# url-kaist/Quatro

Hardware: NVIDIA H100
Metric: registrations/sec (64-ring pair) (higher is better)
Workload: dtype f32 (front end, match, graph filter) / f64 (graph boundary, GNC, COTE)

## Files before the change

quatro_b200/capi.py:

```python
from __future__ import annotations

import ctypes as C
from typing import Optional, Sequence

import numpy as np

from . import _build

PMC_EXACT, PMC_HEU, KCORE_HEU, INLIER_NONE = 0, 1, 2, 3
FLAG_CLIQUE_TRUNCATED = 1
FLAG_LISTS_TRUNCATED = 2
COTE_MEDIAN, COTE_WEIGHTED_MEAN = 0, 1
MEM_HOST, MEM_DEVICE = 0, 1

STATUS_NAMES = {0: "OK", 1: "DEGENERATE_CLIQUE", 2: "DEGENERATE_INPUT", 3: "CAPACITY_EXCEEDED", -1: "ERR_BAD_ARG",
                -2: "ERR_NO_DEVICE", -3: "ERR_CUDA", -4: "ERR_UNSUPPORTED", -5: "ERR_VOXEL_OVERFLOW"}


class Params(C.Structure):
    _fields_ = [
        ("voxel_size", C.c_float), ("normal_radius", C.c_float), ("fpfh_radius", C.c_float), ("grid_cell", C.c_float),
        ("tuple_scale", C.c_float), ("use_crosscheck", C.c_int32), ("use_tuple_test", C.c_int32),
        ("tuple_trials_per_corr", C.c_int32), ("skip_flagged", C.c_int32), ("reserved0", C.c_int32),
        ("seed", C.c_uint64),
# ... 946 lines not shown
    def register_batch_raw(self, pair_array, n: int, params: Params, kind: int, out: np.ndarray):
        return self._check(self.lib.qb200_register_batch(self.h, pair_array, n, C.byref(params), kind, _ptr(out)), "qb200_register_batch")

    def register_batch_enqueue_raw(self, pair_array, n: int, params: Params, kind: int, out: np.ndarray):
        return self._check(self.lib.qb200_register_batch_enqueue(self.h, pair_array, n, C.byref(params), kind, _ptr(out)), "qb200_register_batch_enqueue")

    def register_batch_flush(self):
        return self._check(self.lib.qb200_register_batch_flush(self.h), "qb200_register_batch_flush")

    def last_clique(self, cap: int = 1 << 16):
        idx = np.zeros(cap, np.int32)
        n = C.c_int32(0)
        self._check(self.lib.qb200_get_last_clique(self.h, _ptr(idx), cap, C.byref(n)), "qb200_get_last_clique")
        return idx[: n.value].copy()

    def last_final_inliers(self, cap: int = 1 << 16):
        idx = np.zeros(cap, np.int32)
        n = C.c_int32(0)
        self._check(self.lib.qb200_get_last_final_inliers(self.h, _ptr(idx), cap, C.byref(n)), "qb200_get_last_final_inliers")
        return idx[: n.value].copy()

    def last_correspondences(self, cap: int = 1 << 16):
        corr = np.zeros((cap, 2), np.int32)
        sm = np.zeros((cap, 4), np.float32)
        tm = np.zeros((cap, 4), np.float32)
        n = C.c_int32(0)
        self._check(self.lib.qb200_get_last_correspondences(self.h, _ptr(corr), _ptr(sm), _ptr(tm), cap, C.byref(n)),
                    "qb200_get_last_correspondences")
        return corr[: n.value].copy(), sm[: n.value].copy(), tm[: n.value].copy()

    def debug_match_stats(self, reset: bool = True) -> dict:
        out = np.zeros(4, np.uint64)
        self._check(self.lib.qb200_debug_match_stats(self.h, _ptr(out), int(reset)), "qb200_debug_match_stats")
        return {"exact_evals": int(out[0]), "tiles": int(out[1]), "warmups": int(out[2]), "aborted_stripes": int(out[3])}

    def debug_nn_tables(self, n_src: int, n_tgt: int):
        rb, cb = np.full(n_src, ~np.uint64(0)), np.full(n_tgt, ~np.uint64(0))
        self._check(self.lib.qb200_debug_nn_tables(self.h, _ptr(rb), n_src, _ptr(cb), n_tgt), "qb200_debug_nn_tables")
        return rb, cb

    def debug_tc_profile(self, reset: bool = True) -> np.ndarray:
        out = np.zeros(24, np.uint64)
        self._check(self.lib.qb200_debug_tc_profile(self.h, _ptr(out), int(reset)), "qb200_debug_tc_profile")
        return out

    def debug_tc_footprint(self) -> dict:
        out = np.zeros(5, np.int32)
        self._check(self.lib.qb200_debug_tc_footprint(self.h, _ptr(out)), "qb200_debug_tc_footprint")
        return {"threads": int(out[0]), "dyn_smem": int(out[1]), "static_smem": int(out[2]), "regs": int(out[3]),
                "ctas_per_sm": int(out[4])}

    def debug_match_verify(self, reset: bool = True) -> dict:
        out = np.zeros(2, np.uint64)
        self._check(self.lib.qb200_debug_match_verify(self.h, _ptr(out), int(reset)), "qb200_debug_match_verify")
        return {"compared": int(out[0]), "mismatches": int(out[1])}

    def debug_tc_distances(self, a33, b33) -> np.ndarray:
        a33, b33 = _f32(a33, 33), _f32(b33, 33)
        out = np.zeros((128, 128), np.float32)
        self._check(self.lib.qb200_debug_tc_distances(self.h, _ptr(a33), len(a33), _ptr(b33), len(b33), _ptr(out)), "qb200_debug_tc_distances")
        return out[: len(a33), : len(b33)].copy()

    def kernel_ms(self):
        ms = np.zeros(2, np.float32)
        calls = np.zeros(2, np.int32)
        self.lib.qb200_get_kernel_ms(self.h, _ptr(ms), _ptr(calls), 2)
        return ms, calls
# ... 6 lines not shown
```

quatro_b200/csrc/common.cuh:

```cuda
#pragma once
#include <cuda_runtime.h>
#include <stdint.h>
#include <stdio.h>

#include "quatro_b200.h"

namespace qb {

constexpr int kOffIJ = 1 << 17;
constexpr int kOffK = 1 << 15;
constexpr uint64_t kCellMask = (1ull << 52) - 1;
constexpr uint64_t kCellInvalid = kCellMask;
constexpr int kCloudShift = 52;

__host__ __device__ __forceinline__ bool cell_ok(int i, int j, int k) {
  return i >= -kOffIJ && i < kOffIJ - 1 && j >= -kOffIJ && j < kOffIJ - 1 && k >= -kOffK && k < kOffK - 1;
}
__host__ __device__ __forceinline__ uint64_t cell_key(int i, int j, int k) {
  return ((uint64_t)(k + kOffK) << 36) | ((uint64_t)(j + kOffIJ) << 18) | (uint64_t)(i + kOffIJ);
}

constexpr int kVoxShift = 31;
constexpr uint64_t kVoxMask = (1ull << kVoxShift) - 1;
constexpr uint64_t kVoxInvalid = kVoxMask;
constexpr int kVsChunks = 64;
constexpr int kVsTile = 2048;

__device__ __forceinline__ bool raw_point_kept(const float4 p, int skip_flagged) {
  return isfinite(p.x) && isfinite(p.y) && isfinite(p.z) && !(skip_flagged && p.w < 0.0f);
}
__host__ __device__ __forceinline__ int vox_chunk_size(int n) { return n > 0 ? (n + kVsChunks - 1) / kVsChunks : 1; }

constexpr int kDescDim = 33;
constexpr int kDescPad = 36;
constexpr int kDescK = 40;
constexpr int kMatchTile = 128;
constexpr int kNbrGlobalCap = 80;

struct WaveCounters {
  int* n_valid;
  int* n_vox;
  int* n_lat;
  int* n_cells;
  int* cloud_status;
  int* bbox;
  int* vox_digits;
  int* n_mutual;
  int* n_corr;
  int* swapped;
  int* n_clique;
  int* max_core;
  int* n_final;
  int* flags;
  long long* n_edges;
};

#define QB_CUDA_TRY(h, expr)                                                                    \
  do {                                                                                          \
    cudaError_t _e = (expr);                                                                    \
    if (_e != cudaSuccess) {                                                                    \
      (h)->fail(__FILE__, __LINE__, cudaGetErrorString(_e));                                    \
      return QB200_ERR_CUDA;                                                                    \
    }                                                                                           \
  } while (0)

__device__ __forceinline__ int float_ordered(float f) {
  const int i = __float_as_int(f);
  return i >= 0 ? i : i ^ 0x7FFFFFFF;
// ... 81 lines not shown
```

quatro_b200/csrc/match.cu:

```cuda
#include <stdlib.h>

#include "handle.cuh"
#include "qb_math.cuh"

namespace qb {

constexpr int kMT = kMatchTile;
constexpr int kMatchThreads = 256;

__device__ __forceinline__ unsigned long long pack_dist(float d, int idx) {
  return ((unsigned long long)__float_as_uint(d) << 32) | (unsigned)idx;
}
__device__ __forceinline__ unsigned long long umin64(unsigned long long a, unsigned long long b) { return a < b ? a : b; }
__device__ __forceinline__ unsigned long long shfl_xor_u64(unsigned long long v, int m) {
  const unsigned lo = __shfl_xor_sync(0xffffffffu, (unsigned)v, m), hi = __shfl_xor_sync(0xffffffffu, (unsigned)(v >> 32), m);
  return ((unsigned long long)hi << 32) | lo;
}

__device__ __forceinline__ void cp_async16(void* smem, const void* gmem) {
  const unsigned s = (unsigned)__cvta_generic_to_shared(smem);
  asm volatile("cp.async.cg.shared.global [%0], [%1], 16;\n" ::"r"(s), "l"(gmem));
}
__device__ __forceinline__ void cp_async_commit() { asm volatile("cp.async.commit_group;\n" ::); }
template <int N>
// ... 29 lines not shown
  load_tile_async(Bs0, B, V, 0);
  cp_async_commit();

  unsigned long long rbest[8];
#pragma unroll
  for (int r = 0; r < 8; ++r) rbest[r] = ~0ull;

  const int n_tiles = (nB + kMT - 1) / kMT;
  for (int jt = 0; jt < n_tiles; ++jt) {
    float(*Bs)[kMT] = (jt & 1) ? Bs1 : Bs0;
    if (jt + 1 < n_tiles) {
      load_tile_async((jt & 1) ? Bs0 : Bs1, B, V, (jt + 1) * kMT);
      cp_async_commit();
      cp_async_wait<1>();
    } else {
      cp_async_wait<0>();
    }
    __syncthreads();

    float acc[8][8];
#pragma unroll
    for (int r = 0; r < 8; ++r)
#pragma unroll
      for (int c = 0; c < 8; ++c) acc[r][c] = 0.0f;
#pragma unroll 3
    for (int d = 0; d < kDescDim; ++d) {
      const float4 a0 = *reinterpret_cast<const float4*>(&As[d][ty * 8]), a1 = *reinterpret_cast<const float4*>(&As[d][ty * 8 + 4]);
      const float4 b0 = *reinterpret_cast<const float4*>(&Bs[d][tx * 8]), b1 = *reinterpret_cast<const float4*>(&Bs[d][tx * 8 + 4]);
      const float a[8] = {a0.x, a0.y, a0.z, a0.w, a1.x, a1.y, a1.z, a1.w};
      const float b[8] = {b0.x, b0.y, b0.z, b0.w, b1.x, b1.y, b1.z, b1.w};
#pragma unroll
      for (int r = 0; r < 8; ++r)
#pragma unroll
        for (int c = 0; c < 8; ++c) {
          const float diff = a[r] - b[c];
          acc[r][c] = __fmaf_rn(diff, diff, acc[r][c]);
        }
    }
    const int cbase = jt * kMT + tx * 8, rbase = r0 + ty * 8;
    unsigned long long cbest[8];
#pragma unroll
    for (int c = 0; c < 8; ++c) cbest[c] = ~0ull;
#pragma unroll
    for (int r = 0; r < 8; ++r) {
      const bool rv = rbase + r < nA;
#pragma unroll
      for (int c = 0; c < 8; ++c) {
        const float dd = acc[r][c];
        const bool ok = rv && (cbase + c < nB) && (dd == dd);
        const unsigned long long pr = ok ? pack_dist(dd, cbase + c) : ~0ull;
        const unsigned long long pc = ok ? pack_dist(dd, rbase + r) : ~0ull;
        rbest[r] = umin64(rbest[r], pr);
        cbest[c] = umin64(cbest[c], pc);
      }
    }
#pragma unroll
    for (int c = 0; c < 8; ++c) cbest[c] = umin64(cbest[c], shfl_xor_u64(cbest[c], 16));
    if ((threadIdx.x & 31) < 16) {
#pragma unroll
      for (int c = 0; c < 8; ++c) colred[warp][tx * 8 + c] = cbest[c];
    }
    __syncthreads();
    if (threadIdx.x < kMT) {
      unsigned long long m = colred[0][threadIdx.x];
#pragma unroll
      for (int w = 1; w < 8; ++w) m = umin64(m, colred[w][threadIdx.x]);
      const int col = jt * kMT + threadIdx.x;
      if (col < nB && m != ~0ull) atomicMin(colbest + (size_t)pair * V + col, m);
    }
  }
// ... 368 lines not shown
```

quatro_b200/csrc/tc_match.cu:

```cuda
#include "handle.cuh"
#include <cstdlib>

namespace qb {

constexpr int kTcM = 128, kTcN = 64;
constexpr int kTcBlk = 64;
constexpr int kTcKB = kDescK / 8;
constexpr int kTcTileBytes = kDescK * kTcBlk * 4;
constexpr int kTileFloats = kDescK * kTcBlk;
constexpr int kTcImages = 3;
constexpr int kTcEpiWarps = 8;
constexpr int kTcThreads = (kTcEpiWarps + 2) * 32;
constexpr int kTcDone = 4;
constexpr int kTcStages = 2;
constexpr int kTcSmemTiles = 256;
constexpr float kTcC = 1.2e-4f;
constexpr float kTcNormMax = 0x1p124f;
constexpr float kTcNormRel = 4.0e-6f;
constexpr int kSpinLimit = 400000;

__device__ __forceinline__ uint32_t smem_u32(const void* p) { return (uint32_t)__cvta_generic_to_shared(p); }

__device__ __forceinline__ uint64_t tc_smem_desc(uint32_t addr) {
  return (uint64_t)((addr & 0x3FFFF) >> 4) | ((uint64_t)((kTcBlk * 16) >> 4) << 16) | ((uint64_t)(128 >> 4) << 32);
}

__device__ __forceinline__ void wgmma_tf32_64x64x8(float (&d)[32], uint64_t adesc, uint64_t bdesc, int accumulate) {
  asm volatile(
      "{\n\t"
      ".reg .pred p;\n\t"
      "setp.ne.b32 p, %34, 0;\n\t"
      "wgmma.mma_async.sync.aligned.m64n64k8.f32.tf32.tf32 "
      "{%0, %1, %2, %3, %4, %5, %6, %7, %8, %9, %10, %11, %12, %13, %14, %15, "
      "%16, %17, %18, %19, %20, %21, %22, %23, %24, %25, %26, %27, %28, %29, %30, %31}, %32, %33, p, 1, 1;\n\t"
      "}\n"
      : "+f"(d[0]), "+f"(d[1]), "+f"(d[2]), "+f"(d[3]), "+f"(d[4]), "+f"(d[5]), "+f"(d[6]), "+f"(d[7]), "+f"(d[8]), "+f"(d[9]),
        "+f"(d[10]), "+f"(d[11]), "+f"(d[12]), "+f"(d[13]), "+f"(d[14]), "+f"(d[15]), "+f"(d[16]), "+f"(d[17]), "+f"(d[18]),
        "+f"(d[19]), "+f"(d[20]), "+f"(d[21]), "+f"(d[22]), "+f"(d[23]), "+f"(d[24]), "+f"(d[25]), "+f"(d[26]), "+f"(d[27]),
        "+f"(d[28]), "+f"(d[29]), "+f"(d[30]), "+f"(d[31])
      : "l"(adesc), "l"(bdesc), "r"(accumulate)
      : "memory");
}

__device__ __forceinline__ bool wg_all(bool v, int g) {
  uint32_t r;
  asm volatile(
      "{\n\t.reg .pred p, q;\n\t"
      "setp.ne.u32 p, %1, 0;\n\t"
      "bar.red.and.pred q, %2, 128, p;\n\t"
      "selp.u32 %0, 1, 0, q;\n\t}\n"
      : "=r"(r)
      : "r"((uint32_t)v), "r"(1 + g)
// ... 119 lines not shown
  else rowbest[(size_t)pair * V + q] = rowbest_u[(size_t)pair * V + u];
}

__device__ __forceinline__ void mbar_init(uint32_t bar, int count) {
  asm volatile("mbarrier.init.shared::cta.b64 [%0], %1;\n" ::"r"(bar), "r"(count) : "memory");
}
__device__ __forceinline__ void mbar_expect_tx(uint32_t bar, uint32_t bytes) {
  asm volatile("mbarrier.arrive.expect_tx.shared::cta.b64 _, [%0], %1;\n" ::"r"(bar), "r"(bytes) : "memory");
}
__device__ __forceinline__ void bulk_g2s(uint32_t dst, const void* src, uint32_t bytes, uint32_t bar) {
  asm volatile("cp.async.bulk.shared::cluster.global.mbarrier::complete_tx::bytes [%0], [%1], %2, [%3];\n" ::"r"(dst), "l"(src), "r"(bytes),
               "r"(bar)
               : "memory");
}
__device__ __forceinline__ bool mbar_wait(uint32_t bar, uint32_t parity) {
  for (int spin = 0; spin < kSpinLimit; ++spin) {
    uint32_t ok;
    asm volatile(
        "{\n\t.reg .pred p;\n\t"
        "mbarrier.try_wait.parity.shared::cta.b64 p, [%1], %2;\n\t"
        "selp.u32 %0, 1, 0, p;\n\t}\n"
        : "=r"(ok)
        : "r"(bar), "r"(parity)
        : "memory");
    if (ok) return true;
  }
  return false;
}

__device__ __forceinline__ unsigned long long tc_pack(float d, int idx) {
  return ((unsigned long long)__float_as_uint(d) << 32) | (unsigned)idx;
}

__device__ __forceinline__ void mbar_arrive(uint32_t bar) {
  asm volatile("mbarrier.arrive.shared::cta.b64 _, [%0];\n" ::"r"(bar) : "memory");
}
__device__ __forceinline__ unsigned tc_fkey(float f) {
  unsigned key = __float_as_uint(f);
  key = (key & 0x80000000u) ? ~key : (key | 0x80000000u);
  return f == f ? key : 0xFFFFFFFFu;
}
__device__ __forceinline__ float tc_fkey_inv(unsigned key) { return __uint_as_float((key & 0x80000000u) ? (key & 0x7FFFFFFFu) : ~key); }

template <bool kDbg, bool kProf = false>
__global__ void __launch_bounds__(kTcThreads, 2)
tc_nn_kernel(const float* __restrict__ tiles, const float* __restrict__ norm, const int* __restrict__ n_vox, int V,
             const uint32_t* __restrict__ perm, unsigned long long* __restrict__ rowbest, unsigned long long* __restrict__ colbest_r,
             unsigned* __restrict__ tile_cmax, int* __restrict__ fallback, unsigned long long* __restrict__ stats,
             float* __restrict__ dbg_tile) {
  extern __shared__ __align__(128) unsigned char smem[];
  __shared__ uint64_t s_fullx[kTcStages], s_sfree[kTcStages], s_fullhl, s_mma[kTcDone], s_afull;
  __shared__ unsigned long long s_rbest[kTcM];
  __shared__ __align__(16) float s_wcj[kTcEpiWarps][kTcN];
  __shared__ unsigned short s_queue[kTcEpiWarps][32];
  __shared__ int s_seq[8];
  __shared__ float s_tlb[kTcSmemTiles];
  __shared__ int s_dead, s_abort, s_evals, s_warm, s_npos;
  __shared__ int s_ndec;

  const int pair = blockIdx.y, stripe = blockIdx.x;
  const int cloudA = 2 * pair, cloudB = 2 * pair + 1;
  const int nA = n_vox[cloudA], nB = n_vox[cloudB];
  const int r0 = stripe * kTcM;
  if (r0 >= nA || nB <= 0) return;

  const int warp = threadIdx.x >> 5, lane = threadIdx.x & 31;
  const int NB = V / kTcBlk;
  auto tick = [&]() -> long long { return kProf ? clock64() : 0ll; };
  auto prof = [&](int slot, long long cyc) { if (kProf && lane == 0) atomicAdd(stats + slot, (unsigned long long)cyc); };
  const long long t_begin = tick();
  constexpr uint32_t kABytes = (kTcM / kTcBlk) * kTcImages * kTcTileBytes;
  constexpr uint32_t kHLBytes = 2 * kTcTileBytes;
  constexpr uint32_t kXBytes = kTcTileBytes;
  const uint32_t sA = smem_u32(smem), sHL = sA + kABytes, sX0 = sHL + kHLBytes;
  const float* __restrict__ tA = tiles + (size_t)cloudA * NB * kTcImages * kTileFloats;
  const float* __restrict__ tB = tiles + (size_t)cloudB * NB * kTcImages * kTileFloats;
  const float* __restrict__ nrmA = norm + (size_t)cloudA * V;
  const float* __restrict__ nrmB = norm + (size_t)cloudB * V;
  const uint32_t* __restrict__ permA = perm + (size_t)cloudA * V;
  const uint32_t* __restrict__ permB = perm + (size_t)cloudB * V;
  unsigned long long* __restrict__ cbg = colbest_r + (size_t)pair * V;
  const uint32_t bar_fullx0 = smem_u32(&s_fullx[0]), bar_sfree0 = smem_u32(&s_sfree[0]), bar_fullhl = smem_u32(&s_fullhl),
                 bar_mma0 = smem_u32(&s_mma[0]), bar_a = smem_u32(&s_afull);
  const int n_tiles = (nB + kTcN - 1) / kTcN;

  if (threadIdx.x == 0) {
    for (int i = 0; i < kTcStages; ++i) { mbar_init(bar_fullx0 + 8 * i, 1); mbar_init(bar_sfree0 + 8 * i, kTcEpiWarps); }
    mbar_init(bar_fullhl, 1);
    for (int i = 0; i < kTcDone; ++i) mbar_init(bar_mma0 + 8 * i, kTcEpiWarps);
    mbar_init(bar_a, 1);
    s_dead = 0; s_abort = 0; s_evals = 0; s_warm = 0; s_npos = 0; s_ndec = 0;
    asm volatile("fence.mbarrier_init.release.cluster;\n" ::: "memory");
  }
  if (threadIdx.x < kTcM) s_rbest[threadIdx.x] = ~0ull;
  __syncthreads();
  const long long t_setup = tick();
  if (kProf && threadIdx.x == 0) { atomicAdd(stats + 8, 1ull); atomicAdd(stats + 10, (unsigned long long)(t_setup - t_begin)); }
  volatile int* v_dead = &s_dead;
  volatile int* v_abort = &s_abort;
  volatile int* v_seq = s_seq;
  volatile int* v_ndec = &s_ndec;
  auto wait_decided = [&](int n) -> bool {
    for (int spin = 0; spin < kSpinLimit; ++spin) {
      if (*v_ndec > n) { __threadfence_block(); return true; }
      __nanosleep(32);
    }
    return false;
  };
  volatile unsigned long long* v_rbest = s_rbest;

  if (warp == kTcEpiWarps) {
    auto issue_hl = [&](int n) {
      const int t = v_seq[n & 7];
      if (lane != 0) return;
      if (t < 0) { mbar_arrive(bar_fullhl); return; }
      mbar_expect_tx(bar_fullhl, kHLBytes);
      bulk_g2s(sHL, tB + (size_t)t * kTcImages * kTileFloats, kHLBytes, bar_fullhl);
    };
    if (lane == 0) {
      mbar_expect_tx(bar_a, kABytes);
      bulk_g2s(sA, tA + (size_t)stripe * (kTcM / kTcBlk) * kTcImages * kTileFloats, kABytes, bar_a);
    }
    bool ok = wait_decided(0);
    if (ok) issue_hl(0);
    long long p_wm = 0, p_wd = 0;
    bool ended = !ok || v_seq[0] < 0;
    for (int k = 0; ok && !ended; ++k) {
// ... 9 lines not shown
    }
    prof(12, p_wm); prof(28, p_wd);
    if (!ok) *v_dead = 1;
  } else if (warp == kTcEpiWarps + 1) {
    const float amin = sqrtf(nrmA[r0]), amax = sqrtf(nrmA[(r0 + kTcM < nA ? r0 + kTcM : nA) - 1]);
    auto tile_lb = [&](int t) -> float {
      const float bmin = sqrtf(nrmB[t * kTcN]), bmax = sqrtf(nrmB[(t * kTcN + kTcN < nB ? t * kTcN + kTcN : nB) - 1]);
      const float gap = fmaxf(amin - bmax, bmin - amax) - (2.0e-3f + kTcNormRel * (amax + bmax));
      if (!(amin <= amax && bmin <= bmax)) return 0.0f;
      return gap > 0.0f ? gap * gap * 0.9999f : 0.0f;
    };
    constexpr int kPq = kTcSmemTiles / 32;
    const uint2* __restrict__ tcm2 = reinterpret_cast<const uint2*>(tile_cmax) + (size_t)pair * (V / kTcN);
    uint2 pq[kPq];
    auto fetch_tcm = [&]() {
#pragma unroll
      for (int i = 0; i < kPq; ++i) pq[i] = lane + 32 * i < n_tiles ? __ldcg(tcm2 + lane + 32 * i) : make_uint2(0xFFFFFFFFu, 0xFFFFFFFFu);
    };
    fetch_tcm();
    int t0 = 0;
    {
      float best = INFINITY;
      for (int t = lane; t < n_tiles; t += 32) {
        const float g = tile_lb(t);
        if (t < kTcSmemTiles) s_tlb[t] = g;
        if (g < best) { best = g; t0 = t; }
      }
      const unsigned key = __reduce_min_sync(0xffffffffu, tc_fkey(best));
      const unsigned who = __ballot_sync(0xffffffffu, tc_fkey(best) == key);
      t0 = __shfl_sync(0xffffffffu, t0, __ffs(who) - 1);
      __syncwarp();
    }
    auto tlb = [&](int t) -> float { return t < kTcSmemTiles ? s_tlb[t] : tile_lb(t); };
    int lo = t0 - 1, hi = t0 + 1;
    bool first = true, done = false;
    auto next_tile = [&]() -> int {
      if (first) { first = false; return t0; }
      unsigned rmax = 0;
#pragma unroll
      for (int i = 0; i < kTcM / 32; ++i) {
        const int row = lane + 32 * i;
        if (r0 + row < nA) {
          const unsigned long long rb = v_rbest[row];
          rmax = max(rmax, rb == ~0ull ? 0x7F800000u : (unsigned)(rb >> 32));
        }
      }
      const float rmaxf = __uint_as_float(__reduce_max_sync(0xffffffffu, rmax));
      unsigned tcm[kPq];
#pragma unroll
      for (int i = 0; i < kPq; ++i) tcm[i] = max(pq[i].x, pq[i].y);
      if (*v_abort || *v_dead) return -1;
      const bool is_left = lane < 16;
      while (true) {
        if (lo < 0 && hi >= n_tiles) return -1;
        const int t = is_left ? lo - lane : hi + (lane - 16);
        const bool valid = is_left ? t >= 0 : t < n_tiles;
        const float lb = valid ? tlb(t) : INFINITY;
        unsigned cm = 0xFFFFFFFFu;
        {
          const int src = t & 31, sl = (t >> 5) & (kPq - 1);
#pragma unroll
          for (int i = 0; i < kPq; ++i) {
            const unsigned a = __shfl_sync(0xffffffffu, tcm[i], src);
            if (sl == i) cm = a;
          }
          if (!valid) cm = 0xFFFFFFFFu;
          else if (t >= kTcSmemTiles) { const uint2 q = __ldcg(tcm2 + t); cm = max(q.x, q.y); }
        }
        const bool visit = valid && (lb <= 0.0f || !(lb > rmaxf) || !(lb > __uint_as_float(cm)));
        const unsigned vb = __ballot_sync(0xffffffffu, visit);
// ... 2 lines not shown
        if (fl == 16 && fr == 16) { lo -= 16; hi += 16; continue; }
        const float gl = __shfl_sync(0xffffffffu, lb, fl & 15), gh = __shfl_sync(0xffffffffu, lb, 16 + (fr & 15));
        const bool left = fr == 16 || (fl < 16 && gl <= gh);
        const int tv = left ? lo - fl : hi + fr;
        lo -= left ? fl + 1 : fl;
        hi += left ? fr : fr + 1;
        return tv;
      }
    };
    int n_issued = 0;
    auto decide = [&](int n) {
      int t = -1;
      if (!done) {
        t = next_tile();
        if (t < 0) done = true; else ++n_issued;
      }
      if (lane == 0) {
        v_seq[n & 7] = t;
        __threadfence_block();
        *v_ndec = n + 1;
      }
      __syncwarp();
      if (!done) fetch_tcm();
      return t;
    };
    auto issue_x = [&](int n) {
      const int t = v_seq[n & 7];
      if (lane != 0) return;
      const uint32_t bar = bar_fullx0 + 8 * (n % kTcStages);
      if (t < 0) { mbar_arrive(bar); return; }
      mbar_expect_tx(bar, kXBytes);
      bulk_g2s(sX0 + (n % kTcStages) * kXBytes, tB + ((size_t)t * kTcImages + 2) * kTileFloats, kXBytes, bar);
    };
    for (int n = 0; n < 3; ++n) {
      decide(n);
      if (n < kTcStages) issue_x(n);
    }
    prof(11, tick() - t_setup);
    long long p_wm = 0, p_dec = 0, p_sf = 0;
    auto mbar_test = [&](uint32_t bar, uint32_t parity) -> bool {
      uint32_t ready;
      asm volatile(
          "{\n\t.reg .pred p;\n\t"
          "mbarrier.test_wait.parity.shared::cta.b64 p, [%1], %2;\n\t"
          "selp.u32 %0, 1, 0, p;\n\t}\n"
          : "=r"(ready)
          : "r"(bar), "r"(parity)
          : "memory");
      return __all_sync(0xffffffffu, ready != 0);
    };
    int nd = 3, nx = kTcStages;
    bool ok = true, end_decided = v_seq[0] < 0 || v_seq[1] < 0 || v_seq[2] < 0;
    int idle = 0;
    long long t_idle = 0;
    while (ok && !(end_decided && nx == nd)) {
      const uint32_t bar_s = bar_sfree0 + 8 * (nx % kTcStages), par_s = (uint32_t)((nx / kTcStages - 1) & 1);
      const uint32_t bar_m = bar_mma0 + 8 * ((nd - 3) & (kTcDone - 1)), par_m = (uint32_t)(((nd - 3) >> 2) & 1);
      const bool can_x = nx < nd, can_d = !end_decided && nd < nx + 4;
      if (can_x && mbar_test(bar_s, par_s)) {
        if (kProf && idle) { (can_d ? p_wm : p_sf) += tick() - t_idle; }
        idle = 0;
        issue_x(nx);
        ++nx;
        continue;
      }
      if (can_d && mbar_test(bar_m, par_m)) {
        const long long t1 = tick();
        if (kProf && idle) { (can_x ? p_wm : p_sf) += t1 - t_idle; }
        idle = 0;
        if (decide(nd) < 0) end_decided = true;
        ++nd;
        p_dec += tick() - t1;
        continue;
      }
      if (idle == 0) t_idle = tick();
      if (++idle > kSpinLimit) { ok = false; break; }
      __nanosleep(32);
    }
    prof(29, p_wm); prof(13, p_dec); prof(14, p_sf);
    if (!ok) *v_dead = 1;
    if (lane == 0) s_npos = n_issued;
  } else {
    const int wg = warp >> 2;
    const int rbase = wg * 64 + 16 * (warp & 3);
    const int cl = 2 * (lane & 3);
    const float kLow = 1.0f - 0.5f * kTcC;
    const float kW = kTcC / kLow;
    bool row_ok[2];
    float nam[2], Ri_ub[2];
    unsigned oa[2];
#pragma unroll
    for (int h = 0; h < 2; ++h) {
      const int gi = r0 + rbase + (lane >> 2) + 8 * h;
      row_ok[h] = gi < nA;
      nam[h] = row_ok[h] ? kLow * nrmA[gi] : INFINITY;
      oa[h] = row_ok[h] ? permA[gi] : 0u;
      Ri_ub[h] = row_ok[h] ? INFINITY : -INFINITY;
    }
    const uint32_t row_bits = (row_ok[0] ? 0x33333333u : 0u) | (row_ok[1] ? 0xCCCCCCCCu : 0u);
    const float4* __restrict__ aex = reinterpret_cast<const float4*>(smem + (wg * kTcImages + 2) * kTcTileBytes);
    const uint32_t aH = sA + (uint32_t)(wg * kTcImages * kTcTileBytes), aL = aH + kTcTileBytes;
    float* wcj = s_wcj[warp];
    unsigned short* wq = s_queue[warp];
    int evals_w = 0;
    bool alive = mbar_wait(bar_a, 0);
    const long long t_loop = tick();
    prof(19, t_loop - t_setup);
    long long p_wx = 0, p_wmm = 0, p_ld = 0, p_prep = 0, p_fil = 0, p_ev = 0;
    int p_tiles = 0;
    int pf_tile = -1;
    unsigned long long pf_cb[2] = {~0ull, ~0ull};
    unsigned pf_ob[2] = {0u, 0u};
    unsigned* __restrict__ tcmw = tile_cmax + ((size_t)pair * (V / kTcN)) * 2;
    int rr_tile = -1;
    unsigned rr_val[2] = {0u, 0u};
    auto rr_flush = [&]() {
      if (rr_tile < 0) return;
#pragma unroll
      for (int s = 0; s < 2; ++s) {
        const unsigned m = __reduce_max_sync(0xffffffffu, rr_val[s]);
        if (lane == 0) atomicMin(tcmw + (size_t)rr_tile * 2 + s, m);
      }
      rr_tile = -1;
    };
    for (int k = 0;; ++k) {
      const int ts = k & (kTcDone - 1), st = k % kTcStages;
      const long long q0 = tick();
      if (alive) alive = mbar_wait(bar_fullx0 + 8 * st, (uint32_t)((k / kTcStages) & 1));
      const long long q1 = tick();
      p_wx += q1 - q0;
// ... 38 lines not shown
        break;
      }
      float d[32];
#pragma unroll
      for (int i = 0; i < 32; ++i) d[i] = 0.0f;
      {
        constexpr uint32_t kKB = 2 * kTcBlk * 16;
        const uint32_t bH = sHL, bL = bH + kTcTileBytes;
        asm volatile("wgmma.fence.sync.aligned;\n" ::: "memory");
#pragma unroll
        for (int kb = 0; kb < kTcKB; ++kb) {
          wgmma_tf32_64x64x8(d, tc_smem_desc(aH + kb * kKB), tc_smem_desc(bL + kb * kKB), kb > 0);
          wgmma_tf32_64x64x8(d, tc_smem_desc(aL + kb * kKB), tc_smem_desc(bH + kb * kKB), 1);
        }
#pragma unroll
        for (int kb = 0; kb < kTcKB; ++kb) wgmma_tf32_64x64x8(d, tc_smem_desc(aH + kb * kKB), tc_smem_desc(bH + kb * kKB), 1);
        asm volatile("wgmma.commit_group.sync.aligned;\n" ::: "memory");
        asm volatile("wgmma.wait_group.sync.aligned 0;\n" ::: "memory");
#pragma unroll
        for (int i = 0; i < 32; ++i) asm volatile("" : "+f"(d[i])::"memory");
      }
      __syncwarp();
      if (lane == 0) mbar_arrive(bar_mma0 + 8 * ts);
      const long long q3 = tick();
      p_wmm += q3 - q2;
      p_prep += q2 - q1;
      ++p_tiles;
      const bool skip = __any_sync(0xffffffffu, (*v_abort | *v_dead) != 0);
      const long long q4 = tick();
      p_ld += q4 - q3;
      if (!skip) {
        const float4* __restrict__ bex = reinterpret_cast<const float4*>(smem + kABytes + kHLBytes + st * kXBytes);
        float dbest[2];
        bool col_warm = false;
#pragma unroll
        for (int s = 0; s < 2; ++s) {
          const float nbm = bex[9 * kTcBlk + 32 * s + lane].x;
          dbest[s] = cb_cur[s] == ~0ull ? INFINITY : __uint_as_float((unsigned)(cb_cur[s] >> 32));
          wcj[32 * s + lane] = nbm == INFINITY ? -INFINITY : dbest[s];
          col_warm |= cb_cur[s] == ~0ull && nbm != INFINITY;
        }
        float Ri[2];
        bool row_warm = false;
#pragma unroll
        for (int h = 0; h < 2; ++h) {
          const unsigned long long rb = v_rbest[rbase + (lane >> 2) + 8 * h];
          Ri[h] = fminf(Ri_ub[h], rb == ~0ull ? INFINITY : __uint_as_float((unsigned)(rb >> 32)));
          row_warm |= row_ok[h] && Ri[h] == INFINITY;
        }
        __syncwarp();
        if (__any_sync(0xffffffffu, row_warm || col_warm)) {
          if (lane == 0) atomicAdd(&s_warm, 1);
          float rowub[2] = {INFINITY, INFINITY};
#pragma unroll
          for (int i = 0; i < 32; i += 4) {
#pragma unroll
            for (int e = 0; e < 2; ++e) {
              const int c = 2 * i + cl + e;
              const float nbc = bex[9 * kTcBlk + c].x;
              const float ub0 = fmaf(kW, nam[0] + nbc, d[i + e]), ub1 = fmaf(kW, nam[1] + nbc, d[i + 2 + e]);
              rowub[0] = fminf(rowub[0], ub0);
              rowub[1] = fminf(rowub[1], ub1);
              unsigned mn = min(ub0 >= 0.0f ? __float_as_uint(ub0) : 0xFFFFFFFFu, ub1 >= 0.0f ? __float_as_uint(ub1) : 0xFFFFFFFFu);
              mn = min(mn, __shfl_xor_sync(0xffffffffu, mn, 4));
              mn = min(mn, __shfl_xor_sync(0xffffffffu, mn, 8));
              mn = min(mn, __shfl_xor_sync(0xffffffffu, mn, 16));
              if (lane < 4 && mn != 0xFFFFFFFFu && nbc != INFINITY) wcj[c] = fminf(wcj[c], __uint_as_float(mn));
            }
          }
#pragma unroll
          for (int h = 0; h < 2; ++h) {
            rowub[h] = fminf(rowub[h], __shfl_xor_sync(0xffffffffu, rowub[h], 1));
            rowub[h] = fminf(rowub[h], __shfl_xor_sync(0xffffffffu, rowub[h], 2));
            if (row_ok[h]) { Ri_ub[h] = fminf(Ri_ub[h], rowub[h]); Ri[h] = fminf(Ri[h], Ri_ub[h]); }
          }
        }
        __syncwarp();
        const long long q5 = tick();
        p_prep += q5 - q4;
        const int ncol = nB - c0;
        uint32_t mask = 0, col_bits = 0;
#pragma unroll
        for (int i = 0; i < 32; i += 4) {
          const float2 x = *reinterpret_cast<const float2*>(wcj + 2 * i + cl);
#pragma unroll
          for (int e = 0; e < 4; ++e) {
            const float lbv = d[i + e];
            const float xc = (e & 1) ? x.y : x.x;
            asm("{\n\t.reg .pred p, q;\n\t"
                "setp.le.f32 p, %1, %2;\n\t"
                "setp.le.or.f32 q, %1, %3, p;\n\t"
                "@q or.b32 %0, %0, %4;\n\t}\n"
                : "+r"(mask)
                : "f"(lbv), "f"(xc), "f"(Ri[e >> 1]), "r"(1u << (i + e)));
            if (2 * i + cl + (e & 1) < ncol) col_bits |= 1u << (i + e);
            if (kDbg) {
              const int h = e >> 1, c = 2 * i + cl + (e & 1);
              if (stripe == 0 && row_ok[h] && c < ncol)
                dbg_tile[(size_t)oa[h] * 128 + permB[c0 + c]] = fmaf(0.5f * kW, nam[h] + bex[9 * kTcBlk + c].x, lbv);
            }
          }
        }
        mask &= col_bits & row_bits;
        int remaining = __reduce_add_sync(0xffffffffu, __popc(mask));
        const long long q6 = tick();
        p_fil += q6 - q5;
        evals_w += remaining;
        while (remaining > 0) {
          int tot;
          int p = warp_excl_scan(__popc(mask), &tot);
          while (mask && p < 32) {
            const int i = __ffs(mask) - 1;
            mask &= mask - 1;
            wq[p++] = (unsigned short)((lane << 5) | i);
          }
          __syncwarp();
          const int nb = tot < 32 ? tot : 32;
          const int q = lane < nb ? wq[lane] : 0;
          const int sl = q >> 5, i = q & 31, h = (i >> 1) & 1;
          const int rr = rbase + (sl >> 2) + 8 * h;
          const int c = 8 * (i >> 2) + 2 * (sl & 3) + (i & 1);
          float acc = 0.0f;
#pragma unroll
          for (int kc = 0; kc < (kDescDim + 3) / 4; ++kc) {
            const float4 a = aex[kc * kTcBlk + (rr & (kTcBlk - 1))], b = bex[kc * kTcBlk + c];
            float diff = a.x - b.x;
            acc = __fmaf_rn(diff, diff, acc);
            if (4 * kc + 1 < kDescDim) { diff = a.y - b.y; acc = __fmaf_rn(diff, diff, acc); }
            if (4 * kc + 2 < kDescDim) { diff = a.z - b.z; acc = __fmaf_rn(diff, diff, acc); }
            if (4 * kc + 3 < kDescDim) { diff = a.w - b.w; acc = __fmaf_rn(diff, diff, acc); }
          }
          const float db0 = __shfl_sync(0xffffffffu, dbest[0], c & 31), db1 = __shfl_sync(0xffffffffu, dbest[1], c & 31);
          const unsigned ob0 = __shfl_sync(0xffffffffu, ob[0], c & 31), ob1 = __shfl_sync(0xffffffffu, ob[1], c & 31);
          const unsigned oa0 = __shfl_sync(0xffffffffu, oa[0], sl & ~3), oa1 = __shfl_sync(0xffffffffu, oa[1], sl & ~3);
          const float dbc = c < 32 ? db0 : db1;
          const unsigned oc = c < 32 ? ob0 : ob1;
          const unsigned orow = h ? oa1 : oa0;
          if (lane < nb && acc == acc) {
            const unsigned long long pr = tc_pack(acc, (int)oc);
            if (pr < v_rbest[rr]) atomicMin(&s_rbest[rr], pr);
            if (acc <= dbc) atomicMin(cbg + c0 + c, tc_pack(acc, (int)orow));
          }
          __syncwarp();
          remaining = tot - nb;
        }
        if (lane == 0 && evals_w) {
          const int seen = atomicAdd(&s_evals, evals_w) + evals_w;
          if ((k + 1) * (kTcM * kTcN) >= 8 * 128 * 128 && seen > (k + 1) * (kTcM * kTcN / 2)) *v_abort = 1;
        }
        evals_w = 0;
        p_ev += tick() - q6;
      }
      __syncwarp();
      if (lane == 0) mbar_arrive(bar_sfree0 + 8 * st);
      rr_flush();
      if (!skip) {
        rr_tile = jt;
#pragma unroll
        for (int s = 0; s < 2; ++s) {
          rr_val[s] = 0;
          if (c0 + 32 * s + lane < nB) {
            const unsigned long long cbn = __ldcg(cbg + c0 + 32 * s + lane);
            rr_val[s] = cbn == ~0ull ? 0x7F800000u : (unsigned)(cbn >> 32);
          }
        }
      }
    }
    rr_flush();
    prof(20, p_wx); prof(21, p_wmm); prof(22, p_ld); prof(23, p_prep); prof(24, p_fil); prof(25, p_ev);
    prof(26, tick() - t_loop); prof(27, p_tiles);
  }
  __syncthreads();
  const bool aborted = (s_abort | s_dead) != 0;
  if (kProf && threadIdx.x == 0) atomicAdd(stats + 9, (unsigned long long)(tick() - t_begin));
  if (threadIdx.x == 0) {
    atomicAdd(stats + 0, (unsigned long long)s_evals);
    atomicAdd(stats + 1, (unsigned long long)s_npos);
    atomicAdd(stats + 2, (unsigned long long)s_warm);
    if (aborted) {
      atomicAdd(stats + 3, 1ull);
      fallback[pair] = 1;
    }
  }
  if (!aborted && threadIdx.x < kTcM && r0 + (int)threadIdx.x < nA) rowbest[(size_t)pair * V + r0 + threadIdx.x] = s_rbest[threadIdx.x];
}

static size_t tc_smem_bytes() {
  return ((size_t)(kTcM / kTcBlk) * kTcImages + 2 + kTcStages) * kTcTileBytes;
}

static int tc_prepare(Lane* h, const void* kernel) {
  QB_CUDA_TRY(h, ensure_dyn_smem(h->device, kernel, tc_smem_bytes()));
  QB_CUDA_TRY(h, cudaFuncSetAttribute(kernel, cudaFuncAttributePreferredSharedMemoryCarveout, cudaSharedmemCarveoutMaxShared));
  return QB200_OK;
}

int tc_footprint(Lane* h, int* out5) {
  const void* kernel = (const void*)tc_nn_kernel<false>;
  if (int rc = tc_prepare(h, kernel)) return rc;
  cudaFuncAttributes fa;
  QB_CUDA_TRY(h, cudaFuncGetAttributes(&fa, kernel));
  int ctas = 0;
  QB_CUDA_TRY(h, cudaOccupancyMaxActiveBlocksPerMultiprocessor(&ctas, kernel, kTcThreads, tc_smem_bytes()));
  out5[0] = kTcThreads;
  out5[1] = (int)tc_smem_bytes();
  out5[2] = (int)fa.sharedSizeBytes;
  out5[3] = fa.numRegs;
  out5[4] = ctas;
  return QB200_OK;
}

// ... 1 lines not shown
  const int V = h->V;
  const dim3 g((V + 255) / 256, n_clouds);
  norm_key_kernel<<<g, 256, 0, h->stream>>>(h->desc_t, h->ctr.n_vox, V, h->key_a, h->val_a);
  h->launches += 1;
  int bits = 0;
  while ((1 << bits) < n_clouds) ++bits;
  int rc = launch_cloud_sort(h, n_clouds, h->ctr.n_vox, 32, 32);
  if (rc == QB200_ERR_UNSUPPORTED) rc = sort_pairs(h, n_clouds * V, 32 + bits);
  if (rc) return rc;
  dedup_kernel<<<n_clouds, 1024, 0, h->stream>>>(h->desc_t, h->ctr.n_vox, V, h->key_b, h->val_b, dedup, h->val_a, h->class_of(), h->n_unique());
  h->launches += 1;
  QB_CUDA_TRY(h, cudaGetLastError());
  return QB200_OK;
}

int launch_match_nn(Lane* h, int n_pairs) {
  const int V = h->V;
  const size_t smem = tc_smem_bytes();
  if (int rc = tc_prepare(h, (const void*)tc_nn_kernel<false>)) return rc;
  int rc = sort_and_dedup(h, 2 * n_pairs, 1);
  if (rc) return rc;
  const uint32_t* uperm = h->val_a;
  const uint32_t* class_of = h->class_of();
  const int* n_unique = h->n_unique();
  unsigned long long* colbest_u = h->colpart_col();
  unsigned long long* rowbest_u = h->colpart_row();
  unsigned* tile_cmax = h->colpart_tile_cmax();
  QB_CUDA_TRY(h, cudaMemsetAsync(h->rowbest, 0xFF, (size_t)n_pairs * V * 8, h->stream));
  QB_CUDA_TRY(h, cudaMemsetAsync(h->colbest, 0xFF, (size_t)n_pairs * V * 8, h->stream));
  QB_CUDA_TRY(h, cudaMemsetAsync(h->colpart, 0xFF, h->colpart_count() * 8, h->stream));
  QB_CUDA_TRY(h, cudaMemsetAsync(h->tc_fallback, 0, (size_t)n_pairs * sizeof(int), h->stream));
  const dim3 gsplit((V + 255) / 256, 2 * n_pairs);
  split_desc_kernel<<<gsplit, 256, 0, h->stream>>>(h->desc_t, n_unique, V, uperm, h->desc_tiles, h->desc_norm, h->tc_fallback);
  const dim3 g(h->NS, n_pairs);
  cudaEventRecord(h->kev[0], h->stream);
  if (h->tc_prof) {
    if (int rc2 = tc_prepare(h, (const void*)tc_nn_kernel<false, true>)) return rc2;
    tc_nn_kernel<false, true><<<g, kTcThreads, smem, h->stream>>>(h->desc_tiles, h->desc_norm, n_unique, V, uperm, rowbest_u, colbest_u,
                                                                  tile_cmax, h->tc_fallback, h->tc_stats, nullptr);
  } else {
    tc_nn_kernel<false><<<g, kTcThreads, smem, h->stream>>>(h->desc_tiles, h->desc_norm, n_unique, V, uperm, rowbest_u, colbest_u,
                                                            tile_cmax, h->tc_fallback, h->tc_stats, nullptr);
  }
  cudaEventRecord(h->kev[1], h->stream);
  h->kev_armed[0] = 1;
  broadcast_best_kernel<<<gsplit, 256, 0, h->stream>>>(rowbest_u, colbest_u, h->ctr.n_vox, V, h->val_b, class_of, h->rowbest, h->colbest);
  h->launches += 3;
  QB_CUDA_TRY(h, cudaGetLastError());
  return launch_match_exact(h, n_pairs, h->tc_fallback);
}

int launch_tc_debug_tile(Lane* h, float* d_out) {
  const size_t smem = tc_smem_bytes();
  if (int rc0 = tc_prepare(h, (const void*)tc_nn_kernel<true>)) return rc0;
  int rc = sort_and_dedup(h, 2, 0);
  if (rc) return rc;
  const uint32_t* uperm = h->val_a;
  const int* n_unique = h->n_unique();
  QB_CUDA_TRY(h, cudaMemsetAsync(h->colpart, 0xFF, h->colpart_count() * 8, h->stream));
  QB_CUDA_TRY(h, cudaMemsetAsync(h->tc_fallback, 0, sizeof(int), h->stream));
  const dim3 gsplit((h->V + 255) / 256, 2);
  split_desc_kernel<<<gsplit, 256, 0, h->stream>>>(h->desc_t, n_unique, h->V, uperm, h->desc_tiles, h->desc_norm, h->tc_fallback);
  const dim3 g(1, 1);
  tc_nn_kernel<true><<<g, kTcThreads, smem, h->stream>>>(h->desc_tiles, h->desc_norm, n_unique, h->V, uperm, h->colpart_row(), h->colpart_col(),
                                                         h->colpart_tile_cmax(), h->tc_fallback, h->tc_stats, d_out);
  h->launches += 2;
  QB_CUDA_TRY(h, cudaGetLastError());
  return QB200_OK;
}

}
```

Measured before the change: 14240.

## Seed NN bounds with norm-sorted window search before tensor-core match

Adds a pre-pass kernel that, for each descriptor, binary-searches the other cloud's norm-sorted list and computes exact distances to a small window of neighbours. This seeds the row-best, column-best and tile max tables before the tensor-core NN kernel runs. The main kernel now loads the seeded row bests, and the per-tile warm-up upper-bound path and its first-tile special case are removed, which should tighten pruning from the start. The cost is one extra launch and a small amount of exact-distance work per point, and the early pruning now relies on seed quality.

```diff
diff --git a/quatro_b200/capi.py b/quatro_b200/capi.py
--- a/quatro_b200/capi.py
+++ b/quatro_b200/capi.py
@@ -1002,7 +1002,7 @@
     def debug_match_stats(self, reset: bool = True) -> dict:
         out = np.zeros(4, np.uint64)
         self._check(self.lib.qb200_debug_match_stats(self.h, _ptr(out), int(reset)), "qb200_debug_match_stats")
-        return {"exact_evals": int(out[0]), "tiles": int(out[1]), "warmups": int(out[2]), "aborted_stripes": int(out[3])}
+        return {"exact_evals": int(out[0]), "tiles": int(out[1]), "aborted_stripes": int(out[3])}
 
     def debug_nn_tables(self, n_src: int, n_tgt: int):
         rb, cb = np.full(n_src, ~np.uint64(0)), np.full(n_tgt, ~np.uint64(0))
diff --git a/quatro_b200/csrc/common.cuh b/quatro_b200/csrc/common.cuh
--- a/quatro_b200/csrc/common.cuh
+++ b/quatro_b200/csrc/common.cuh
@@ -34,6 +34,10 @@
 constexpr int kDescDim = 33;
 constexpr int kDescPad = 36;
 constexpr int kDescK = 40;
+__device__ __forceinline__ float desc_dist_step(float acc, float a, float b) {
+  const float diff = a - b;
+  return __fmaf_rn(diff, diff, acc);
+}
 constexpr int kMatchTile = 128;
 constexpr int kNbrGlobalCap = 80;
 
diff --git a/quatro_b200/csrc/match.cu b/quatro_b200/csrc/match.cu
--- a/quatro_b200/csrc/match.cu
+++ b/quatro_b200/csrc/match.cu
@@ -85,10 +85,7 @@
 #pragma unroll
       for (int r = 0; r < 8; ++r)
 #pragma unroll
-        for (int c = 0; c < 8; ++c) {
-          const float diff = a[r] - b[c];
-          acc[r][c] = __fmaf_rn(diff, diff, acc[r][c]);
-        }
+        for (int c = 0; c < 8; ++c) acc[r][c] = desc_dist_step(acc[r][c], a[r], b[c]);
     }
     const int cbase = jt * kMT + tx * 8, rbase = r0 + ty * 8;
     unsigned long long cbest[8];
diff --git a/quatro_b200/csrc/tc_match.cu b/quatro_b200/csrc/tc_match.cu
--- a/quatro_b200/csrc/tc_match.cu
+++ b/quatro_b200/csrc/tc_match.cu
@@ -18,6 +18,7 @@
 constexpr float kTcNormMax = 0x1p124f;
 constexpr float kTcNormRel = 4.0e-6f;
 constexpr int kSpinLimit = 400000;
+constexpr int kSeedW = 16;
 
 __device__ __forceinline__ uint32_t smem_u32(const void* p) { return (uint32_t)__cvta_generic_to_shared(p); }
 
@@ -203,6 +204,61 @@
   return ((unsigned long long)__float_as_uint(d) << 32) | (unsigned)idx;
 }
 
+template <class FA, class FB>
+__device__ __forceinline__ float tc_exact_dist(FA a, FB b) {
+  float acc = 0.0f;
+#pragma unroll
+  for (int kc = 0; kc < (kDescDim + 3) / 4; ++kc) {
+    const float4 x = a(kc), y = b(kc);
+    acc = desc_dist_step(acc, x.x, y.x);
+    if (4 * kc + 1 < kDescDim) acc = desc_dist_step(acc, x.y, y.y);
+    if (4 * kc + 2 < kDescDim) acc = desc_dist_step(acc, x.z, y.z);
+    if (4 * kc + 3 < kDescDim) acc = desc_dist_step(acc, x.w, y.w);
+  }
+  return acc;
+}
+
+__global__ void __launch_bounds__(256) tc_seed_kernel(const float* __restrict__ tiles, const float* __restrict__ norm,
+                                                      const int* __restrict__ n_vox, int V, const uint32_t* __restrict__ perm,
+                                                      const int* __restrict__ fallback, unsigned long long* __restrict__ rowbest,
+                                                      unsigned long long* __restrict__ colbest, unsigned* __restrict__ tile_cmax) {
+  const int cloud = blockIdx.y, pair = cloud >> 1, other = cloud ^ 1;
+  const int r = blockIdx.x * blockDim.x + threadIdx.x;
+  const int n = n_vox[cloud], no = n_vox[other];
+  if (fallback[pair] || (r & ~(kTcN - 1)) >= n) return;
+  const int NB = V / kTcBlk;
+  auto image = [&](int c, int q) {
+    return reinterpret_cast<const float4*>(tiles + ((size_t)(c * NB + q / kTcBlk) * kTcImages + 2) * kTileFloats) + q % kTcBlk;
+  };
+  unsigned long long best = ~0ull;
+  if (r < n && no > 0) {
+    const float4* __restrict__ ia = image(cloud, r);
+    float4 own[(kDescDim + 3) / 4];
+#pragma unroll
+    for (int kc = 0; kc < (kDescDim + 3) / 4; ++kc) own[kc] = ia[kc * kTcBlk];
+    const float* __restrict__ nrm = norm + (size_t)other * V;
+    const float key = norm[(size_t)cloud * V + r];
+    int lo = 0, hi = no;
+    while (lo < hi) {
+      const int mid = (lo + hi) >> 1;
+      if (nrm[mid] < key) lo = mid + 1; else hi = mid;
+    }
+    const int j1 = min(no, lo + kSeedW);
+    for (int j = max(0, lo - kSeedW); j < j1; ++j) {
+      const float4* __restrict__ ib = image(other, j);
+      const float d = tc_exact_dist([&](int kc) { return own[kc]; }, [&](int kc) { return ib[kc * kTcBlk]; });
+      if (d == d) best = min(best, tc_pack(d, (int)perm[(size_t)other * V + j]));
+    }
+  }
+  if (cloud & 1) {
+    if (r < n) colbest[(size_t)pair * V + r] = best;
+    const unsigned m = __reduce_max_sync(0xffffffffu, r < n ? (unsigned)(best >> 32) : 0u);
+    if ((threadIdx.x & 31) == 0) tile_cmax[((size_t)pair * (V / kTcN) + r / kTcN) * 2 + ((r / 32) & 1)] = m;
+  } else if (r < n) {
+    rowbest[(size_t)pair * V + r] = best;
+  }
+}
+
 __device__ __forceinline__ void mbar_arrive(uint32_t bar) {
   asm volatile("mbarrier.arrive.shared::cta.b64 _, [%0];\n" ::"r"(bar) : "memory");
 }
@@ -226,7 +282,7 @@
   __shared__ unsigned short s_queue[kTcEpiWarps][32];
   __shared__ int s_seq[8];
   __shared__ float s_tlb[kTcSmemTiles];
-  __shared__ int s_dead, s_abort, s_evals, s_warm, s_npos;
+  __shared__ int s_dead, s_abort, s_evals, s_npos;
   __shared__ int s_ndec;
 
   const int pair = blockIdx.y, stripe = blockIdx.x;
@@ -260,10 +316,10 @@
     mbar_init(bar_fullhl, 1);
     for (int i = 0; i < kTcDone; ++i) mbar_init(bar_mma0 + 8 * i, kTcEpiWarps);
     mbar_init(bar_a, 1);
-    s_dead = 0; s_abort = 0; s_evals = 0; s_warm = 0; s_npos = 0; s_ndec = 0;
+    s_dead = 0; s_abort = 0; s_evals = 0; s_npos = 0; s_ndec = 0;
     asm volatile("fence.mbarrier_init.release.cluster;\n" ::: "memory");
   }
-  if (threadIdx.x < kTcM) s_rbest[threadIdx.x] = ~0ull;
+  if (threadIdx.x < kTcM) s_rbest[threadIdx.x] = r0 + (int)threadIdx.x < nA ? rowbest[(size_t)pair * V + r0 + threadIdx.x] : ~0ull;
   __syncthreads();
   const long long t_setup = tick();
   if (kProf && threadIdx.x == 0) { atomicAdd(stats + 8, 1ull); atomicAdd(stats + 10, (unsigned long long)(t_setup - t_begin)); }
@@ -339,10 +395,9 @@
       __syncwarp();
     }
     auto tlb = [&](int t) -> float { return t < kTcSmemTiles ? s_tlb[t] : tile_lb(t); };
-    int lo = t0 - 1, hi = t0 + 1;
-    bool first = true, done = false;
+    int lo = t0, hi = t0 + 1;
+    bool done = false;
     auto next_tile = [&]() -> int {
-      if (first) { first = false; return t0; }
       unsigned rmax = 0;
 #pragma unroll
       for (int i = 0; i < kTcM / 32; ++i) {
@@ -411,10 +466,11 @@
       mbar_expect_tx(bar, kXBytes);
       bulk_g2s(sX0 + (n % kTcStages) * kXBytes, tB + ((size_t)t * kTcImages + 2) * kTileFloats, kXBytes, bar);
     };
-    for (int n = 0; n < 3; ++n) {
-      decide(n);
-      if (n < kTcStages) issue_x(n);
-    }
+    int nd = 0;
+    bool end_decided = false;
+    while (nd < 3 && !end_decided) end_decided = decide(nd++) < 0;
+    int nx = 0;
+    while (nx < kTcStages && nx < nd) issue_x(nx++);
     prof(11, tick() - t_setup);
     long long p_wm = 0, p_dec = 0, p_sf = 0;
     auto mbar_test = [&](uint32_t bar, uint32_t parity) -> bool {
@@ -428,8 +484,7 @@
           : "memory");
       return __all_sync(0xffffffffu, ready != 0);
     };
-    int nd = 3, nx = kTcStages;
-    bool ok = true, end_decided = v_seq[0] < 0 || v_seq[1] < 0 || v_seq[2] < 0;
+    bool ok = true;
     int idle = 0;
     long long t_idle = 0;
     while (ok && !(end_decided && nx == nd)) {
@@ -466,7 +521,7 @@
     const float kLow = 1.0f - 0.5f * kTcC;
     const float kW = kTcC / kLow;
     bool row_ok[2];
-    float nam[2], Ri_ub[2];
+    float nam[2];
     unsigned oa[2];
 #pragma unroll
     for (int h = 0; h < 2; ++h) {
@@ -474,7 +529,6 @@
       row_ok[h] = gi < nA;
       nam[h] = row_ok[h] ? kLow * nrmA[gi] : INFINITY;
       oa[h] = row_ok[h] ? permA[gi] : 0u;
-      Ri_ub[h] = row_ok[h] ? INFINITY : -INFINITY;
     }
     const uint32_t row_bits = (row_ok[0] ? 0x33333333u : 0u) | (row_ok[1] ? 0xCCCCCCCCu : 0u);
     const float4* __restrict__ aex = reinterpret_cast<const float4*>(smem + (wg * kTcImages + 2) * kTcTileBytes);
@@ -579,48 +633,17 @@
       if (!skip) {
         const float4* __restrict__ bex = reinterpret_cast<const float4*>(smem + kABytes + kHLBytes + st * kXBytes);
         float dbest[2];
-        bool col_warm = false;
 #pragma unroll
         for (int s = 0; s < 2; ++s) {
           const float nbm = bex[9 * kTcBlk + 32 * s + lane].x;
           dbest[s] = cb_cur[s] == ~0ull ? INFINITY : __uint_as_float((unsigned)(cb_cur[s] >> 32));
           wcj[32 * s + lane] = nbm == INFINITY ? -INFINITY : dbest[s];
-          col_warm |= cb_cur[s] == ~0ull && nbm != INFINITY;
         }
         float Ri[2];
-        bool row_warm = false;
 #pragma unroll
         for (int h = 0; h < 2; ++h) {
           const unsigned long long rb = v_rbest[rbase + (lane >> 2) + 8 * h];
-          Ri[h] = fminf(Ri_ub[h], rb == ~0ull ? INFINITY : __uint_as_float((unsigned)(rb >> 32)));
-          row_warm |= row_ok[h] && Ri[h] == INFINITY;
-        }
-        __syncwarp();
-        if (__any_sync(0xffffffffu, row_warm || col_warm)) {
-          if (lane == 0) atomicAdd(&s_warm, 1);
-          float rowub[2] = {INFINITY, INFINITY};
-#pragma unroll
-          for (int i = 0; i < 32; i += 4) {
-#pragma unroll
-            for (int e = 0; e < 2; ++e) {
-              const int c = 2 * i + cl + e;
-              const float nbc = bex[9 * kTcBlk + c].x;
-              const float ub0 = fmaf(kW, nam[0] + nbc, d[i + e]), ub1 = fmaf(kW, nam[1] + nbc, d[i + 2 + e]);
-              rowub[0] = fminf(rowub[0], ub0);
-              rowub[1] = fminf(rowub[1], ub1);
-              unsigned mn = min(ub0 >= 0.0f ? __float_as_uint(ub0) : 0xFFFFFFFFu, ub1 >= 0.0f ? __float_as_uint(ub1) : 0xFFFFFFFFu);
-              mn = min(mn, __shfl_xor_sync(0xffffffffu, mn, 4));
-              mn = min(mn, __shfl_xor_sync(0xffffffffu, mn, 8));
-              mn = min(mn, __shfl_xor_sync(0xffffffffu, mn, 16));
-              if (lane < 4 && mn != 0xFFFFFFFFu && nbc != INFINITY) wcj[c] = fminf(wcj[c], __uint_as_float(mn));
-            }
-          }
-#pragma unroll
-          for (int h = 0; h < 2; ++h) {
-            rowub[h] = fminf(rowub[h], __shfl_xor_sync(0xffffffffu, rowub[h], 1));
-            rowub[h] = fminf(rowub[h], __shfl_xor_sync(0xffffffffu, rowub[h], 2));
-            if (row_ok[h]) { Ri_ub[h] = fminf(Ri_ub[h], rowub[h]); Ri[h] = fminf(Ri[h], Ri_ub[h]); }
-          }
+          Ri[h] = rb == ~0ull ? INFINITY : __uint_as_float((unsigned)(rb >> 32));
         }
         __syncwarp();
         const long long q5 = tick();
@@ -667,16 +690,8 @@
           const int sl = q >> 5, i = q & 31, h = (i >> 1) & 1;
           const int rr = rbase + (sl >> 2) + 8 * h;
           const int c = 8 * (i >> 2) + 2 * (sl & 3) + (i & 1);
-          float acc = 0.0f;
-#pragma unroll
-          for (int kc = 0; kc < (kDescDim + 3) / 4; ++kc) {
-            const float4 a = aex[kc * kTcBlk + (rr & (kTcBlk - 1))], b = bex[kc * kTcBlk + c];
-            float diff = a.x - b.x;
-            acc = __fmaf_rn(diff, diff, acc);
-            if (4 * kc + 1 < kDescDim) { diff = a.y - b.y; acc = __fmaf_rn(diff, diff, acc); }
-            if (4 * kc + 2 < kDescDim) { diff = a.z - b.z; acc = __fmaf_rn(diff, diff, acc); }
-            if (4 * kc + 3 < kDescDim) { diff = a.w - b.w; acc = __fmaf_rn(diff, diff, acc); }
-          }
+          const float acc = tc_exact_dist([&](int kc) { return aex[kc * kTcBlk + (rr & (kTcBlk - 1))]; },
+                                          [&](int kc) { return bex[kc * kTcBlk + c]; });
           const float db0 = __shfl_sync(0xffffffffu, dbest[0], c & 31), db1 = __shfl_sync(0xffffffffu, dbest[1], c & 31);
           const unsigned ob0 = __shfl_sync(0xffffffffu, ob[0], c & 31), ob1 = __shfl_sync(0xffffffffu, ob[1], c & 31);
           const unsigned oa0 = __shfl_sync(0xffffffffu, oa[0], sl & ~3), oa1 = __shfl_sync(0xffffffffu, oa[1], sl & ~3);
@@ -723,7 +738,6 @@
   if (threadIdx.x == 0) {
     atomicAdd(stats + 0, (unsigned long long)s_evals);
     atomicAdd(stats + 1, (unsigned long long)s_npos);
-    atomicAdd(stats + 2, (unsigned long long)s_warm);
     if (aborted) {
       atomicAdd(stats + 3, 1ull);
       fallback[pair] = 1;
@@ -791,6 +805,7 @@
   QB_CUDA_TRY(h, cudaMemsetAsync(h->tc_fallback, 0, (size_t)n_pairs * sizeof(int), h->stream));
   const dim3 gsplit((V + 255) / 256, 2 * n_pairs);
   split_desc_kernel<<<gsplit, 256, 0, h->stream>>>(h->desc_t, n_unique, V, uperm, h->desc_tiles, h->desc_norm, h->tc_fallback);
+  tc_seed_kernel<<<gsplit, 256, 0, h->stream>>>(h->desc_tiles, h->desc_norm, n_unique, V, uperm, h->tc_fallback, rowbest_u, colbest_u, tile_cmax);
   const dim3 g(h->NS, n_pairs);
   cudaEventRecord(h->kev[0], h->stream);
   if (h->tc_prof) {
@@ -804,7 +819,7 @@
   cudaEventRecord(h->kev[1], h->stream);
   h->kev_armed[0] = 1;
   broadcast_best_kernel<<<gsplit, 256, 0, h->stream>>>(rowbest_u, colbest_u, h->ctr.n_vox, V, h->val_b, class_of, h->rowbest, h->colbest);
-  h->launches += 3;
+  h->launches += 4;
   QB_CUDA_TRY(h, cudaGetLastError());
   return launch_match_exact(h, n_pairs, h->tc_fallback);
 }
@@ -820,10 +835,12 @@
   QB_CUDA_TRY(h, cudaMemsetAsync(h->tc_fallback, 0, sizeof(int), h->stream));
   const dim3 gsplit((h->V + 255) / 256, 2);
   split_desc_kernel<<<gsplit, 256, 0, h->stream>>>(h->desc_t, n_unique, h->V, uperm, h->desc_tiles, h->desc_norm, h->tc_fallback);
+  tc_seed_kernel<<<gsplit, 256, 0, h->stream>>>(h->desc_tiles, h->desc_norm, n_unique, h->V, uperm, h->tc_fallback, h->colpart_row(),
+                                                h->colpart_col(), h->colpart_tile_cmax());
   const dim3 g(1, 1);
   tc_nn_kernel<true><<<g, kTcThreads, smem, h->stream>>>(h->desc_tiles, h->desc_norm, n_unique, h->V, uperm, h->colpart_row(), h->colpart_col(),
                                                          h->colpart_tile_cmax(), h->tc_fallback, h->tc_stats, d_out);
-  h->launches += 2;
+  h->launches += 3;
   QB_CUDA_TRY(h, cudaGetLastError());
   return QB200_OK;
 }
```

Measured after the change: 14730 (median of 6 runs). 3.4% higher.
